# r9y9/deepvoice3_pytorch

Measured on AMD Instinct MI355X. Metric: mel-frames/sec/node (train step, deepvoice3_ljspeech), higher is better.
Workload: dtype f16x3

## Files before the change

deepvoice3_pytorch_amd/csrc/loss.hip:

```cpp
#include "common.h"

namespace {

constexpr int kLossBlock = 256;

__device__ __forceinline__ void block_reduce4(float v[4], float* out ) {
  __shared__ float red[4][4];
#pragma unroll
  for (int k = 0; k < 4; ++k) v[k] = dv3_wave_sum(v[k]);
  const int w = threadIdx.x >> 6;
  if ((threadIdx.x & 63) == 0) {
#pragma unroll
    for (int k = 0; k < 4; ++k) red[w][k] = v[k];
  }
  __syncthreads();
  if (threadIdx.x < 4) out[threadIdx.x] = red[0][threadIdx.x] + red[1][threadIdx.x] +
                                          red[2][threadIdx.x] + red[3][threadIdx.x];
}

template <bool FAST = false>
__device__ __forceinline__ void spec_bd(float yh, float y, float& z, float& dz) {
  const float eps = 1e-8f;
  const float a = yh + eps, b = 1.f - yh + eps;
  constexpr float LN2 = 0.69314718055994530942f;
  const float la = FAST ? __builtin_amdgcn_logf(a) * LN2 : logf(a), lb = FAST ? __builtin_amdgcn_logf(b) * LN2 : logf(b);
  const float ab = a + b;
  z = -y * (la - lb) + ((FAST ? __builtin_amdgcn_logf(ab) * LN2 : logf(ab)) - lb);
  const float ra = __builtin_amdgcn_rcpf(a), rb = __builtin_amdgcn_rcpf(b);
  dz = (a * __builtin_amdgcn_rcpf(ab) - y) * (ra + rb);
}

__device__ __forceinline__ int spec_t_valid(const dv3_spec_loss_desc& p) {
  if (!p.t_valid) return p.T;
  const int tv = p.t_valid[0];
  return tv < p.T ? (tv > p.r ? tv : p.r + 1) : p.T;
}

__device__ __forceinline__ float spec_mask_sum(const dv3_spec_loss_desc& p) {
  float ms = 0.f;
  const int Tr = spec_t_valid(p) - p.r;
  for (int b = 0; b < p.B; ++b) {
    int l = p.lengths[b] - p.r;
    l = l < 0 ? 0 : (l > Tr ? Tr : l);
    ms += (float)l;
  }
  return ms * (float)p.D;
}

__global__ __launch_bounds__(kLossBlock) void spec_loss_kernel(const dv3_spec_loss_desc p) {
  const int Tr = p.T - p.r, D = p.D;
  const int Trv = spec_t_valid(p) - p.r;
  const int64_t n = (int64_t)p.B * Tr * D;
  const bool use_mask = p.w_masked > 0.f && p.lengths;
  const float msum = use_mask ? spec_mask_sum(p) : 1.f;
  const float inv_n = 1.0f / (float)((int64_t)p.B * Trv * D);
  const float wm = use_mask ? p.w_masked : 0.f;
  const float c_all = (1.f - wm) * inv_n, c_msk = use_mask ? wm / msum : 0.f;
  float acc[4] = {0.f, 0.f, 0.f, 0.f};
  const int64_t stride = (int64_t)gridDim.x * kLossBlock;
  const bool t_fast = p.yh_ts < p.yh_ds;
  for (int64_t i = (int64_t)blockIdx.x * kLossBlock + threadIdx.x; i < n; i += stride) {
    int dd, t, b;
    if (t_fast) {
      t = (int)(i % Tr);
      const int64_t bd = i / Tr;
      dd = (int)(bd % D);
      b = (int)(bd / D);
    } else {
      dd = (int)(i % D);
      const int64_t bt = i / D;
      t = (int)(bt % Tr);
      b = (int)(bt / Tr);
    }
    const int64_t ih = b * p.yh_bs + t * p.yh_ts + dd * p.yh_ds;
    const int64_t iy = b * p.y_bs + (int64_t)(t + p.r) * p.y_ts + dd * p.y_ds;
    if (t >= Trv) {
      if (p.dyh) p.dyh[ih] = 0.f;
      continue;
    }
    const float yh = p.y_hat[ih], y = p.y[iy];
    const float m = (use_mask && (t + p.r) < p.lengths[b]) ? 1.f : 0.f;
    const float diff = yh - y;
    const float ad = fabsf(diff);
    acc[0] += ad;
    acc[1] += m * ad;
    float dz = 0.f;
    if (p.w_bd > 0.f) {
      float z;
      spec_bd(yh, y, z, dz);
      acc[2] += z;
      acc[3] += m * z;
    }
    if (p.dyh) {
      const float sgn = (diff > 0.f) ? 1.f : ((diff < 0.f) ? -1.f : 0.f);
      const float coef = c_all + c_msk * m;
      p.dyh[ih] = p.gscale * coef * ((1.f - p.w_bd) * sgn + p.w_bd * dz);
    }
  }
  block_reduce4(acc, p.scratch + (int64_t)blockIdx.x * 4);
}

template <bool FAST>
__global__ __launch_bounds__(kLossBlock) void spec_loss_tiled_kernel(const dv3_spec_loss_desc p, int t_tiles, int d_tiles,
                                                                     int n_tiles) {
  __shared__ float ys[64 * 65];
  const int Tr = p.T - p.r, D = p.D;
  const int Trv = spec_t_valid(p) - p.r;
  const bool use_mask = p.w_masked > 0.f && p.lengths;
  const float msum = use_mask ? spec_mask_sum(p) : 1.f;
  const float inv_n = 1.0f / (float)((int64_t)p.B * Trv * D);
  const float wm = use_mask ? p.w_masked : 0.f;
  const float c_all = (1.f - wm) * inv_n, c_msk = use_mask ? wm / msum : 0.f;
  float acc[4] = {0.f, 0.f, 0.f, 0.f};
  const int tid = threadIdx.x;
  for (int tile = blockIdx.x; tile < n_tiles; tile += gridDim.x) {
    const int dt = tile % d_tiles, tt_ = (tile / d_tiles) % t_tiles, b = tile / (d_tiles * t_tiles);
    const int t0 = tt_ * 64, d0 = dt * 64;
    __syncthreads();
#pragma unroll 4
    for (int q = tid; q < 64 * 64; q += kLossBlock) {
      const int tl = q >> 6, dl = q & 63;
      const int t = t0 + tl, dd = d0 + dl;
      ys[tl * 65 + dl] = (t < Tr && dd < D) ? p.y[b * p.y_bs + (int64_t)(t + p.r) * p.y_ts + dd] : 0.f;
    }
    __syncthreads();
    const int len_b = use_mask ? p.lengths[b] : 0;
#pragma unroll 4
    for (int q = tid; q < 64 * 64; q += kLossBlock) {
      const int dl = q >> 6, tl = q & 63;
      const int t = t0 + tl, dd = d0 + dl;
      if (t >= Tr || dd >= D) continue;
      const int64_t ih = b * p.yh_bs + t + (int64_t)dd * p.yh_ds;
      if (t >= Trv) {
        if (p.dyh) p.dyh[ih] = 0.f;
        continue;
      }
      const float yh = p.y_hat[ih], y = ys[tl * 65 + dl];
      const float m = (use_mask && (t + p.r) < len_b) ? 1.f : 0.f;
      const float diff = yh - y;
      const float ad = fabsf(diff);
      acc[0] += ad;
      acc[1] += m * ad;
      float dz = 0.f;
      if (p.w_bd > 0.f) {
        float z;
        spec_bd<FAST>(yh, y, z, dz);
        acc[2] += z;
        acc[3] += m * z;
      }
      if (p.dyh) {
        const float sgn = (diff > 0.f) ? 1.f : ((diff < 0.f) ? -1.f : 0.f);
        const float coef = c_all + c_msk * m;
        p.dyh[ih] = p.gscale * coef * ((1.f - p.w_bd) * sgn + p.w_bd * dz);
      }
    }
  }
  block_reduce4(acc, p.scratch + (int64_t)blockIdx.x * 4);
}

__global__ __launch_bounds__(256) void spec_loss_tail_zero_kernel(const dv3_spec_loss_desc p) {
  const int64_t n = (int64_t)p.B * p.r * p.D;
  const int64_t i = (int64_t)blockIdx.x * 256 + threadIdx.x;
  if (i >= n) return;
  const int dd = (int)(i % p.D);
  const int64_t bt = i / p.D;
  const int t = p.T - p.r + (int)(bt % p.r);
  const int b = (int)(bt / p.r);
  p.dyh[b * p.yh_bs + t * p.yh_ts + dd * p.yh_ds] = 0.f;
}

__global__ __launch_bounds__(256) void spec_loss_finish_kernel(const dv3_spec_loss_desc p,
                                                               int n_blocks) {
  float acc[4] = {0.f, 0.f, 0.f, 0.f};
  for (int i = threadIdx.x; i < n_blocks; i += 256)
#pragma unroll
    for (int k = 0; k < 4; ++k) acc[k] += p.scratch[(int64_t)i * 4 + k];
  __shared__ float fin[4];
// ... 56 lines not shown
  for (int i = threadIdx.x; i < n_blocks; i += 256) acc[0] += scratch[(int64_t)i * 4];
  __shared__ float fin[4];
  block_reduce4(acc, fin);
  __syncthreads();
  if (threadIdx.x == 0) {
    if (va) {
      int64_t n = count * min(va[0], cap_a);
      if (vb) n *= min(vb[0], cap_b);
      scale = 1.0f / (float)n;
    }
    out1[0] = fin[0] * scale;
  }
}

__device__ __forceinline__ float bce_elem(float x, float y) {
  const float lx = fmaxf(logf(x), -100.f), l1x = fmaxf(logf(1.f - x), -100.f);
  return -(y * lx + (1.f - y) * l1x);
}

__global__ __launch_bounds__(256) void bce_kernel(const float* __restrict__ p,
                                                  const float* __restrict__ t,
                                                  float* __restrict__ dp, float* __restrict__ scratch,
                                                  int64_t n, float gscale, int T = 0,
                                                  const int32_t* __restrict__ t_valid = nullptr) {
  float acc[4] = {0.f, 0.f, 0.f, 0.f};
  const int Tv = t_valid ? min(t_valid[0], T) : T;
  const float inv_n = 1.0f / (float)(t_valid ? (n / T) * Tv : n);
  const int64_t stride = (int64_t)gridDim.x * 256;
  for (int64_t i = (int64_t)blockIdx.x * 256 + threadIdx.x; i < n; i += stride) {
    if (t_valid && (int)(i % T) >= Tv) {
      if (dp) dp[i] = 0.f;
      continue;
    }
    const float x = p[i], y = t[i];
    acc[0] += bce_elem(x, y);
    if (dp) dp[i] = gscale * inv_n * (x - y) / fmaxf((1.f - x) * x, 1e-12f);
  }
  block_reduce4(acc, scratch + (int64_t)blockIdx.x * 4);
}


constexpr int kItemSliceFrames = 64, kItemMaxSlices = 64;

inline int item_slices(int T) {
  const int s = dv3_cdiv(T, kItemSliceFrames);
  return s < 1 ? 1 : (s > kItemMaxSlices ? kItemMaxSlices : s);
}

__device__ __forceinline__ int clamp_len(int l, int cap) { return l < 0 ? 0 : (l > cap ? cap : l); }

__device__ __forceinline__ void item_slice(int n, int& t0, int& t1) {
  const int per = (n + (int)gridDim.x - 1) / (int)gridDim.x;
  t0 = min((int)blockIdx.x * per, n);
  t1 = min(t0 + per, n);
}

template <bool FAST>
__global__ __launch_bounds__(kLossBlock) void spec_items_kernel(const dv3_spec_items_desc p) {
  const int b = blockIdx.y, D = p.D;
  int t0, t1;
  item_slice(clamp_len(p.lengths[b] - p.r, p.T - p.r), t0, t1);
// ... 75 lines not shown
template <class Desc>
inline bool spec_time_fast(const Desc& d) {
  return d.yh_ts == 1 && d.y_ds == 1 && d.yh_ds > 1 && d.y_ts > 1 && (int64_t)d.B * d.yh_bs < (1ll << 40);
}

inline int loss_blocks(int64_t n) {
  int64_t b = dv3_cdiv64(n, (int64_t)kLossBlock * 4);
  if (b < 1) b = 1;
  if (b > 1024) b = 1024;
  return (int)b;
}

}

int g_loss_fast_log = 1;

extern "C" int dv3_spec_loss_scratch_floats(int32_t B, int32_t T, int32_t D) {
  int64_t tiles = (int64_t)B * dv3_cdiv(T, 64) * dv3_cdiv(D, 64);
  if (tiles > 1024) tiles = 1024;
  const int64_t flat = loss_blocks((int64_t)B * T * D);
  return (int)(4 * (tiles > flat ? tiles : flat) + 16);
}

extern "C" int dv3_spec_loss_f32(const dv3_spec_loss_desc* d, void* stream) {
  DV3_REQUIRE(d && d->y_hat && d->y && d->out4 && d->scratch, "spec_loss: null pointer");
  DV3_REQUIRE(d->B > 0 && d->D > 0 && d->r >= 0 && d->T > d->r, "spec_loss: bad dims");
  DV3_REQUIRE(d->w_masked <= 0.f || d->lengths, "spec_loss: masked weight needs lengths");
  hipStream_t st = (hipStream_t)stream;
  const int64_t n = (int64_t)d->B * (d->T - d->r) * d->D;
  int nb = loss_blocks(n);
  if (spec_time_fast(*d)) {
    const int t_tiles = dv3_cdiv(d->T - d->r, 64), d_tiles = dv3_cdiv(d->D, 64);
    const int64_t nt = (int64_t)d->B * t_tiles * d_tiles;
    nb = (int)(nt < 1024 ? nt : 1024);
    if (g_loss_fast_log) hipLaunchKernelGGL(spec_loss_tiled_kernel<true>, dim3(nb), dim3(kLossBlock), 0, st, *d, t_tiles, d_tiles, (int)nt);
    else hipLaunchKernelGGL(spec_loss_tiled_kernel<false>, dim3(nb), dim3(kLossBlock), 0, st, *d, t_tiles, d_tiles, (int)nt);
  } else {
    hipLaunchKernelGGL(spec_loss_kernel, dim3(nb), dim3(kLossBlock), 0, st, *d);
  }
  if (d->dyh && d->r > 0) {
    const int64_t nt = (int64_t)d->B * d->r * d->D;
    hipLaunchKernelGGL(spec_loss_tail_zero_kernel, dim3((unsigned)dv3_cdiv64(nt, 256)), dim3(256), 0,
                       st, *d);
  }
  hipLaunchKernelGGL(spec_loss_finish_kernel, dim3(1), dim3(256), 0, st, *d, nb);
  return dv3_check_launch("spec_loss_f32");
}

extern "C" int dv3_guided_attn_loss_f32(const float* attn, const int32_t* in_len,
                                        const int32_t* out_len, float* dattn, float* out1,
                                        float* scratch, int32_t L, int32_t B, int32_t Tq, int32_t Tk,
                                        float g, float gscale, void* stream) {
  DV3_REQUIRE(attn && in_len && out_len && out1 && scratch, "guided_attn: null pointer");
  DV3_REQUIRE(L > 0 && B > 0 && Tq > 0 && Tk > 0 && g > 0.f, "guided_attn: bad dims");
  hipStream_t st = (hipStream_t)stream;
  const int64_t per = (int64_t)B * Tq * Tk;
  const int nb = loss_blocks(per);
  hipLaunchKernelGGL(guided_attn_kernel, dim3(nb), dim3(256), 0, st, attn, in_len, out_len, dattn,
                     scratch, L, B, Tq, Tk, g, gscale, (const int32_t*)nullptr, (const int32_t*)nullptr);
  hipLaunchKernelGGL(sum_finish_kernel, dim3(1), dim3(256), 0, st, scratch, nb,
                     1.0f / (float)(per * L), out1, (const int32_t*)nullptr, 0, (const int32_t*)nullptr, 0, (int64_t)0);
  return dv3_check_launch("guided_attn_loss_f32");
}

extern "C" int dv3_guided_attn_loss_valid_f32(const float* attn, const int32_t* in_len, const int32_t* out_len,
                                              float* dattn, float* out1, float* scratch, int32_t L, int32_t B,
                                              int32_t Tq, int32_t Tk, float g, float gscale,
                                              const int32_t* tq_valid, const int32_t* tk_valid, void* stream) {
  DV3_REQUIRE(attn && in_len && out_len && out1 && scratch && tq_valid && tk_valid, "guided_attn_valid: null pointer");
// ... 9 lines not shown
}

extern "C" int dv3_bce_loss_f32(const float* p, const float* t, float* dp, float* out1,
                                float* scratch, int64_t n, float gscale, void* stream) {
  DV3_REQUIRE(p && t && out1 && scratch && n > 0, "bce_loss: bad args");
  hipStream_t st = (hipStream_t)stream;
  const int nb = loss_blocks(n);
  hipLaunchKernelGGL(bce_kernel, dim3(nb), dim3(256), 0, st, p, t, dp, scratch, n, gscale, 0, (const int32_t*)nullptr);
  hipLaunchKernelGGL(sum_finish_kernel, dim3(1), dim3(256), 0, st, scratch, nb, 1.0f / (float)n, out1,
                     (const int32_t*)nullptr, 0, (const int32_t*)nullptr, 0, (int64_t)0);
  return dv3_check_launch("bce_loss_f32");
}

extern "C" int dv3_bce_loss_valid_f32(const float* p, const float* t, float* dp, float* out1, float* scratch,
                                      int64_t rows, int32_t T, const int32_t* t_valid, float gscale, void* stream) {
  DV3_REQUIRE(p && t && out1 && scratch && t_valid && rows > 0 && T > 0, "bce_loss_valid: bad args");
  hipStream_t st = (hipStream_t)stream;
  const int64_t n = rows * T;
  const int nb = loss_blocks(n);
  hipLaunchKernelGGL(bce_kernel, dim3(nb), dim3(256), 0, st, p, t, dp, scratch, n, gscale, (int)T, t_valid);
  hipLaunchKernelGGL(sum_finish_kernel, dim3(1), dim3(256), 0, st, scratch, nb, 0.f, out1, t_valid, (int)T,
                     (const int32_t*)nullptr, 0, rows);
  return dv3_check_launch("bce_loss_valid_f32");
}

extern "C" int dv3_loss_items_scratch_floats(int32_t B, int32_t T) {
  if (B <= 0 || T <= 0) return 0;
  return (int)((int64_t)4 * B * item_slices(T));
}

extern "C" int dv3_spec_loss_items_f32(const dv3_spec_items_desc* d, void* stream) {
  DV3_REQUIRE(d && d->y_hat && d->y && d->lengths && d->out && d->scratch, "spec_loss_items: null pointer");
  DV3_REQUIRE(d->B > 0 && d->B <= 65535 && d->D > 0 && d->r >= 0 && d->T > 0, "spec_loss_items: bad dims");
  hipStream_t st = (hipStream_t)stream;
  const int Tr = d->T > d->r ? d->T - d->r : 0;
  const int S = Tr > 0 ? item_slices(Tr) : 0;
  if (S > 0) {
    DV3_REQUIRE((int64_t)dv3_cdiv(Tr, S) * d->D < (1ll << 31), "spec_loss_items: slice too large");
    if (spec_time_fast(*d) && g_loss_fast_log)
      hipLaunchKernelGGL(spec_items_kernel<true>, dim3(S, d->B), dim3(kLossBlock), 0, st, *d);
    else
      hipLaunchKernelGGL(spec_items_kernel<false>, dim3(S, d->B), dim3(kLossBlock), 0, st, *d);
  }
  hipLaunchKernelGGL(items_finish_kernel, dim3(dv3_cdiv(d->B, 256)), dim3(256), 0, st, (const float*)d->scratch, (int)d->B,
                     S, 2, d->out, d->lengths, (int)d->r, Tr, (const int32_t*)nullptr, 0, (int64_t)d->D);
  return dv3_check_launch("spec_loss_items_f32");
// ... 29 lines not shown
```

deepvoice3_pytorch_amd/ops.py:

```python
import contextlib
import ctypes
import functools
import math

import torch

from . import _lib
from ._lib import CONSTS, STRUCTS, _env_flag, _env_int, _env_str

EPI_LINEAR = CONSTS["DV3_EPI_LINEAR"]
EPI_RELU = CONSTS["DV3_EPI_RELU"]
EPI_SIGMOID = CONSTS["DV3_EPI_SIGMOID"]
EPI_GLU = CONSTS["DV3_EPI_GLU"]
EPI_HIGHWAY = CONSTS["DV3_EPI_HIGHWAY"]
EPI_DGRAD = CONSTS["DV3_EPI_DGRAD"]
EPI_SOFTSIGN = CONSTS["DV3_EPI_SOFTSIGN"]
STORE_BCT = CONSTS["DV3_STORE_BCT"]
STORE_INTERLEAVE2 = CONSTS["DV3_STORE_INTERLEAVE2"]

_conv_desc = STRUCTS["dv3_conv_desc"]
_wgrad_desc = STRUCTS["dv3_wgrad_desc"]
_wn_desc = STRUCTS["dv3_wn_desc"]
_wn_bwd_desc = STRUCTS["dv3_wn_bwd_desc"]
_gate_bwd_desc = STRUCTS["dv3_gate_bwd_desc"]
# ... 1030 lines not shown


fuse_gate_bwd = _env_flag("DV3_FUSE_GATE", True)
fuse_gate_max_elems = _env_int("DV3_FUSE_GATE_MAX", 4 << 20)
pair_words = _env_flag("DV3_PAIR_WORDS", True)
gate_fuse_stats = {"fused": 0, "standalone": 0}


class _GateToken(object):
    __slots__ = ("ab", "mode", "residual", "x", "C", "pair")

    def __init__(self, ab, mode, residual, x, C, pair):
        self.ab, self.mode, self.residual, self.x, self.C, self.pair = ab, mode, residual, x, C, pair


class _GateResult(object):
    __slots__ = ("tok", "dab", "dres", "part", "n_part", "pair", "version")

    def __init__(self, tok, gate, version):
        self.tok, self.dab, self.dres, self.part, self.n_part = tok, gate.dab, gate.dres, gate.part, gate.n_part
        self.pair, self.version = gate.pair, version


def mark_sole_consumer(y):
    if fuse_gate_bwd and getattr(y, "_dv3_tok", None) is not None:
        y._dv3_sole = True
    return y


def _spk_strides(spk):
    if spk is None:
        return 0, 0, 0
    if spk.dim() == 2:
        return spk.stride(0), 1, 0
    return spk.stride(0), spk.stride(1), 1


def _grads_in_place(leaves):
    return all(getattr(t, "_dv3_grad_inplace", False) and t.grad is not None and t.requires_grad for t in leaves)


def _grad_inplace_arm(ctx, v, g, bias):
    leaves = [t for t in (v, g, bias) if t is not None]
    ctx.inplace = bool(leaves) and _grads_in_place(leaves)
    ctx.leaves = (v, g, bias) if ctx.inplace else None
    if ctx.inplace:
# ... 86 lines not shown
            raise ValueError("gated layers keep the sequence length")
        ab_dtype = torch.bfloat16 if (_gemm_mode == "bf16" and pk.fwd_s is not None and split_only) else torch.float32
        ab = torch.empty((B, M, T), dtype=ab_dtype, device=x.device) if (gated and need_grad) else None
        if spk is not None:
            spk = _c(spk)
        res_in = x if gated else (_c(r) if r is not None else None)
        r2c = _c(r2) if r2 is not None else None
        y = conv_gemm(x, pk.fwd, pk.lda, pk.a_half, B=B, Cin=Cin, Tin=T, M=M, Tout=Tout,
                      J=J_, dil=cfg.dil, padL=padL, mode=mode, Cg=Cg,
                      bias=bias, spk=spk, spk_strides=_spk_strides(spk),
                      r=res_in if (mode == EPI_HIGHWAY or cfg.residual or not gated) else None,
                      r2=r2c, residual=int(cfg.residual), ab=ab, xmask=bits, xmask_rs=bits_rs, xmask_c8=keep8,
                      drop_scale=dscale, a_split=pk.fwd_s if _gemm_mode != "f32" else None,
                      store_mode=STORE_INTERLEAVE2 if cfg.transposed else STORE_BCT)
        if need_grad:
            _grad_inplace_arm(ctx, v, g, bias)
            ctx.cfg, ctx.pk, ctx.dims = cfg, pk, (B, Cin, T, Tout, M, Cg, J, padL)
            ctx.bits, ctx.bits_rs, ctx.dscale = bits, bits_rs, dscale
            ctx.spk_dim = spk.dim() if spk is not None else 0
            ctx.has_r, ctx.has_r2 = (r is not None), (r2 is not None)
            ctx.has_bias = bias is not None
            ctx.save_for_backward(x, v, g, ab if gated else y)
            ctx.tok = ctx.prod = None
            split_modes = _gemm_mode in ("f16x3", "bf16x3")
            ctx.pair_ok = bool(gated and pair_words and split_modes and pk.bwd_s is not None and
                               split_only and ab.dtype == torch.float32 and (spk is None or spk.dim() == 2) and
                               not (M <= 64 and Cin <= 64))
            if fuse_gate_bwd and split_modes and pk.bwd_s is not None:
                if gated and ab.dtype == torch.float32 and spk is None and split_only and \
                        B * Cg * T <= fuse_gate_max_elems:
                    ctx.tok = _GateToken(ab, mode, int(cfg.residual), x if mode == EPI_HIGHWAY else None, Cg,
                                         pair=ctx.pair_ok)
                    y._dv3_tok = ctx.tok
                prod = getattr(x_in, "_dv3_tok", None) if (x_in is x and getattr(x_in, "_dv3_sole", False)) else None
                if prod is not None and prod.C == Cin and ctx.needs_input_grad[0] and Tout == T and \
                        (J_ - 1) * cfg.dil <= 64 and J_ <= 16:
                    ctx.prod = prod
        return y

    @staticmethod
    def backward(ctx, dy):
        cfg, pk = ctx.cfg, ctx.pk
        B, Cin, T, Tout, M, Cg, J, padL = ctx.dims
        x, v, g, saved = ctx.saved_tensors
        mode = cfg.mode
        gated = mode in (EPI_GLU, EPI_HIGHWAY)
        dy = _c(dy)
        rs2 = math.sqrt(0.5)
        dr = dr2 = dspk = None
        r_scale = 0.0
        n_part, g_pair, part_t = B, False, False
        if gated:
            glu_skip = mode == EPI_GLU and cfg.residual
            fused = getattr(dy, "_dv3_gate", None)
            if fused is not None and ctx.tok is not None and fused.tok is ctx.tok and dy._version == fused.version:
                dab, dres, part = fused.dab, fused.dres, fused.part
                n_part, g_pair, part_t = fused.n_part, fused.pair, True
                dy._dv3_gate = None
                gate_fuse_stats["fused"] += 1
            else:
                g_pair = ctx.pair_ok
                dab, dres, part = gate_bwd(dy, saved, x if mode == EPI_HIGHWAY else None, B=B, C=Cg, T=T,
                                           mode=mode, residual=int(cfg.residual), want_dres=(mode == EPI_HIGHWAY),
                                           pair=g_pair)
                gate_fuse_stats["standalone"] += 1
            if glu_skip:
                dres, r_scale = dy, rs2
            if ctx.spk_dim == 2:
                dspk = part[:, :Cg].contiguous()
            elif ctx.spk_dim == 3:
                dspk = dab[:, :Cg, :]
            gmat, Tg = dab, T
        elif cfg.transposed:
            O = pk.O
            _, _, part = gate_bwd(dy, None, None, B=B, C=O, T=2 * T, mode=EPI_LINEAR, want_dpre=False)
# ... 724 lines not shown
        d.y_bs, d.y_ts, d.y_ds = y.stride()
        d.dyh, d.out4, d.scratch = _ptr(dyh), out4.data_ptr(), scratch.data_ptr()
        d.B, d.T, d.D, d.r = B, T, D, r
        d.w_masked, d.w_bd, d.gscale = w_masked, w_bd, 1.0
        d.t_valid = _ptr(t_valid)
        _lib.call("dv3_spec_loss_f32", ctypes.byref(d), _stream())
        ctx.dyh = dyh
        return out4

    @staticmethod
    def backward(ctx, dout):
        g = ctx.dyh * dout[2] if ctx.dyh is not None else None
        return g, None, None, None, None, None, None


def spec_loss(y_hat, y, lengths, r=1, w_masked=0.5, w_bd=0.1, t_valid=None):
    return SpecLossFn.apply(y_hat, y, lengths, r, w_masked, w_bd, t_valid)


class _NoCtx(object):
    needs_input_grad = (True,)


def spec_loss_with_grad(y_hat, y, lengths, r=1, w_masked=0.5, w_bd=0.1, t_valid=None):
    c = _NoCtx()
    out4 = SpecLossFn.forward(c, y_hat.detach(), y, lengths, r, w_masked, w_bd, t_valid)
    return out4, c.dyh


def guided_attention_loss_with_grad(attn, in_len, out_len, g=0.2, tq_valid=None, tk_valid=None):
    c = _NoCtx()
    out1 = GuidedAttnLossFn.forward(c, attn.detach(), in_len, out_len, g, tq_valid, tk_valid)
    return out1, c.dattn


def bce_loss_with_grad(p, t, t_valid=None):
    c = _NoCtx()
    out1 = BCELossFn.forward(c, p.detach(), t, t_valid)
    return out1, c.dp


def sum_scalars(a, b, c=None, d=None):
    out = torch.empty(1, dtype=torch.float32, device=a.device)
    _lib.call("dv3_sum_scalars_f32", a.data_ptr(), b.data_ptr(), _ptr(c), _ptr(d), out.data_ptr(), _stream())
    return out


def scaled_copy(a, alpha=1.0):
    out = torch.empty_like(a)
    _lib.call("dv3_axpby_f32", a.data_ptr(), None, out.data_ptr(), a.numel(), float(alpha), _stream())
    return out


class GuidedAttnLossFn(torch.autograd.Function):
    @staticmethod
    def forward(ctx, attn, in_len, out_len, g, tq_valid=None, tk_valid=None):
        attn = _c(_chk(attn, "attn"))
        L, B, Tq, Tk = attn.shape
        dev = attn.device
        out1 = torch.empty(1, dtype=torch.float32, device=dev)
        scratch = torch.empty(4 * 1024 + 16, dtype=torch.float32, device=dev)
        dattn = torch.empty_like(attn) if ctx.needs_input_grad[0] else None
# ... 135 lines not shown
```

deepvoice3_pytorch_amd/torch_ops.py:

```python
import math

import torch

from . import ops

_NS = "dv3hip"
_lib = torch.library.Library(_NS, "DEF")

GLU, HIGHWAY = 0, 1
ACT_LINEAR, ACT_RELU, ACT_SIGMOID = 0, 1, 2
_MODES = {GLU: ops.EPI_GLU, HIGHWAY: ops.EPI_HIGHWAY}
_ACTS = {ACT_LINEAR: ops.EPI_LINEAR, ACT_RELU: ops.EPI_RELU, ACT_SIGMOID: ops.EPI_SIGMOID}


class _Ctx(object):

    def __init__(self, needs):
        self.needs_input_grad = tuple(needs)
        self.saved_tensors = ()

    def save_for_backward(self, *tensors):
        self.saved_tensors = tensors


# ... 274 lines not shown

def _attn_backward(ctx, g_ctx, g_P, g_Pd, g_bits):
    q, k, v, P, Pd, bits = ctx.saved_tensors
    if g_ctx is None:
        g_ctx = torch.zeros_like(q)
    dq, dk, dv = torch.ops.dv3hip.attention_bwd(g_ctx.contiguous(), g_P, q, k, v, P, Pd, bits, ctx.p_drop)
    return dq, dk, dv, None, None, None, None


torch.library.register_autograd("dv3hip::attention_fwd", _attn_backward, setup_context=_attn_setup)


_lib.define("sincos_pos_embed(Tensor positions, Tensor table, float w) -> Tensor")
_lib.impl("sincos_pos_embed", lambda positions, table, w: ops.sincos_pos_bct(positions, table, float(w)), "CUDA")
_lib.impl("sincos_pos_embed", lambda positions, table, w: table.new_empty((positions.shape[0], table.shape[1],
                                                                           positions.shape[1])), "Meta")


_lib.define("spec_loss_fwd(Tensor y_hat, Tensor y, Tensor? lengths, int r, float w_masked, float w_bd) "
            "-> (Tensor out4, Tensor grad_y_hat)")
_lib.define("guided_attn_loss_fwd(Tensor attn, Tensor in_lens, Tensor out_lens, float g) -> (Tensor loss, Tensor grad_attn)")
_lib.define("bce_loss_fwd(Tensor p, Tensor target) -> (Tensor loss, Tensor grad_p)")
_lib.impl("spec_loss_fwd", lambda y_hat, y, lengths, r, w_masked, w_bd: ops.spec_loss_with_grad(y_hat, y, lengths, r, w_masked,
                                                                                                 w_bd), "CUDA")
_lib.impl("guided_attn_loss_fwd", lambda attn, il, ol, g: ops.guided_attention_loss_with_grad(attn, il, ol, g), "CUDA")
_lib.impl("bce_loss_fwd", lambda p, t: ops.bce_loss_with_grad(p, t), "CUDA")
_lib.impl("spec_loss_fwd", lambda y_hat, y, lengths, r, w_masked, w_bd: (y_hat.new_empty((4,)), torch.empty_like(y_hat)), "Meta")
_lib.impl("guided_attn_loss_fwd", lambda attn, il, ol, g: (attn.new_empty((1,)), torch.empty_like(attn)), "Meta")
_lib.impl("bce_loss_fwd", lambda p, t: (p.new_empty((1,)), torch.empty_like(p)), "Meta")


def _loss_setup(ctx, inputs, output):
    ctx.save_for_backward(output[1])


def _spec_backward(ctx, g_out4, g_grad):
    (gr,) = ctx.saved_tensors
    return gr * g_out4[2], None, None, None, None, None


def _scalar_backward(n_inputs):
    def backward(ctx, g_loss, g_grad):
        (gr,) = ctx.saved_tensors
        return (gr * g_loss,) + (None,) * (n_inputs - 1)
    return backward


torch.library.register_autograd("dv3hip::spec_loss_fwd", _spec_backward, setup_context=_loss_setup)
torch.library.register_autograd("dv3hip::guided_attn_loss_fwd", _scalar_backward(4), setup_context=_loss_setup)
# ... 44 lines not shown
```

include/dv3hip.h:

```cpp
#ifndef DV3HIP_H
#define DV3HIP_H

#include <stdint.h>

#ifdef __cplusplus
extern "C" {
#endif

#define DV3_OK 0
#define DV3_EINVAL (-1)
#define DV3_ELAUNCH (-2)

#define DV3_ABI_VERSION 49
int dv3_abi_version(void);
const char* dv3_last_error(void);
int dv3_device_info(int dev, char* name, int name_len, int* n_cu);
int dv3_sizeof(const char* name);
int dv3_debug_set(int what, int value);
int dv3_debug_read(int what, void* dst, int64_t bytes);
int dv3_debug_get(int what);

int dv3_ring_standin(const void* src, int64_t src_bytes, void* scratch, int64_t scratch_bytes, int64_t bytes,
                     int32_t channels, int32_t threads, float bytes_per_us, void* stream);

// ... 233 lines not shown
                                 int32_t n_pos, int32_t apply_sincos, void* stream);
int dv3_sincos_pos_bwd_f32(const int64_t* pos, const float* table, const float* w,
                           int32_t w_per_batch, const float* dout, float* dw, int32_t B, int32_t T,
                           int32_t C, int32_t n_pos, void* stream);
int dv3_sincos_pos_bwd2_f32(const int64_t* pos, const float* table, const float* w,
                            int32_t w_per_batch, const float* dout, float* partial, int32_t n_chunks, float* dw,
                            int32_t B, int32_t T, int32_t C, int32_t n_pos, void* stream);
int dv3_shift_append_f32(float* buf, const float* x, int64_t rows, int32_t L, int64_t x_stride,
                         void* stream);
int dv3_ragged_pad_rows_b32(const uint32_t* src, const int32_t* row_off, uint32_t* out, int32_t B,
                            int32_t T_out, int32_t D, int32_t lead, int32_t t_stride, void* stream);
int dv3_deinterleave2_f32(const float* dy, float* out, int32_t B, int32_t O, int32_t T,
                          void* stream);

typedef struct dv3_spec_loss_desc {
  const float* y_hat; const float* y; const int32_t* lengths;
  float* dyh; float* out4; float* scratch;
  int64_t yh_bs, yh_ts, yh_ds;
  int64_t y_bs, y_ts, y_ds;
  int32_t B, T, D, r; float w_masked, w_bd, gscale;
  const int32_t* t_valid;
} dv3_spec_loss_desc;
int dv3_spec_loss_f32(const dv3_spec_loss_desc* d, void* stream);
int dv3_spec_loss_scratch_floats(int32_t B, int32_t T, int32_t D);

int dv3_guided_attn_loss_f32(const float* attn, const int32_t* in_len, const int32_t* out_len,
                             float* dattn, float* out1, float* scratch, int32_t L, int32_t B,
                             int32_t Tq, int32_t Tk, float g, float gscale, void* stream);
int dv3_guided_attn_loss_valid_f32(const float* attn, const int32_t* in_len, const int32_t* out_len,
                                   float* dattn, float* out1, float* scratch, int32_t L, int32_t B,
                                   int32_t Tq, int32_t Tk, float g, float gscale, const int32_t* tq_valid,
                                   const int32_t* tk_valid, void* stream);
int dv3_bce_loss_f32(const float* p, const float* t, float* dp, float* out1, float* scratch,
                     int64_t n, float gscale, void* stream);
int dv3_bce_loss_valid_f32(const float* p, const float* t, float* dp, float* out1, float* scratch,
                           int64_t rows, int32_t T, const int32_t* t_valid, float gscale, void* stream);

typedef struct dv3_spec_items_desc {
  const float* y_hat; const float* y; const int32_t* lengths;
  float* out; float* scratch;
  int64_t yh_bs, yh_ts, yh_ds;
  int64_t y_bs, y_ts, y_ds;
  int32_t B, T, D, r;
} dv3_spec_items_desc;
int dv3_loss_items_scratch_floats(int32_t B, int32_t T);
int dv3_spec_loss_items_f32(const dv3_spec_items_desc* d, void* stream);
int dv3_bce_loss_items_f32(const float* p, const float* t, const int32_t* lengths, float* out, float* scratch,
                           int32_t B, int32_t T, void* stream);
int dv3_guided_attn_loss_items_f32(const float* attn, const int32_t* in_len, const int32_t* out_len, float* out,
                                   float* scratch, int32_t L, int32_t B, int32_t Tq, int32_t Tk, float g,
                                   void* stream);

int dv3_grad_sqnorm_f32(const float* g, int64_t n, float* partial, int32_t n_partial,
                        float* out2, void* stream);
int dv3_clip_adam_f32(float* p, const float* g, float* m, float* v, int64_t n,
                      const float* grad_norm, float clip, const float* hyper, float beta1,
                      float beta2, float eps, float weight_decay, float grad_prescale,
                      void* stream);

// ... 150 lines not shown
```

Baseline: 3.808 million.

## Fuse sigmoid-head backward into spec and BCE loss kernels

Adds head variants of the spectrogram and BCE loss kernels. These compute the gradient with respect to the pre-sigmoid activation directly (dL/dy * y(1-y)) and optionally write per-tile bias partial sums. The sigmoid-epilogue GEMM backward picks up this precomputed gradient through a token, so the standalone dy materialisation and the sigmoid-gate backward pass are skipped. The tiled spec-loss kernel is also restructured to prefetch the next tile into registers while the current one computes. This adds token bookkeeping and a fallback redo path when the upstream gradient is not the placeholder, with extra complexity and risk of silent mismatches.

```diff
diff --git a/deepvoice3_pytorch_amd/csrc/loss.hip b/deepvoice3_pytorch_amd/csrc/loss.hip
--- a/deepvoice3_pytorch_amd/csrc/loss.hip
+++ b/deepvoice3_pytorch_amd/csrc/loss.hip
@@ -4,7 +4,11 @@
 
 constexpr int kLossBlock = 256;
 
-__device__ __forceinline__ void block_reduce4(float v[4], float* out ) {
+struct spec_loss_args : dv3_spec_loss_desc {
+  float* dpre; float* bias_part;
+};
+
+__device__ __forceinline__ void block_reduce4(float v[4], float* out , float* extra = nullptr) {
   __shared__ float red[4][4];
 #pragma unroll
   for (int k = 0; k < 4; ++k) v[k] = dv3_wave_sum(v[k]);
@@ -14,8 +18,16 @@
     for (int k = 0; k < 4; ++k) red[w][k] = v[k];
   }
   __syncthreads();
-  if (threadIdx.x < 4) out[threadIdx.x] = red[0][threadIdx.x] + red[1][threadIdx.x] +
-                                          red[2][threadIdx.x] + red[3][threadIdx.x];
+  if (threadIdx.x < 4) {
+    const float sum = red[0][threadIdx.x] + red[1][threadIdx.x] + red[2][threadIdx.x] + red[3][threadIdx.x];
+    out[threadIdx.x] = sum;
+    if (extra && threadIdx.x == 1) extra[0] = sum;
+  }
+}
+
+__device__ __forceinline__ float sigmoid_head_dz(float dyh, float yh) {
+  const float d = dyh * 1.0f;
+  return d * yh * (1.0f - yh);
 }
 
 template <bool FAST = false>
@@ -47,7 +59,7 @@
   return ms * (float)p.D;
 }
 
-__global__ __launch_bounds__(kLossBlock) void spec_loss_kernel(const dv3_spec_loss_desc p) {
+__global__ __launch_bounds__(kLossBlock) void spec_loss_kernel(const spec_loss_args p) {
   const int Tr = p.T - p.r, D = p.D;
   const int Trv = spec_t_valid(p) - p.r;
   const int64_t n = (int64_t)p.B * Tr * D;
@@ -76,6 +88,7 @@
     const int64_t iy = b * p.y_bs + (int64_t)(t + p.r) * p.y_ts + dd * p.y_ds;
     if (t >= Trv) {
       if (p.dyh) p.dyh[ih] = 0.f;
+      if (p.dpre) p.dpre[ih] = 0.f;
       continue;
     }
     const float yh = p.y_hat[ih], y = p.y[iy];
@@ -91,17 +104,42 @@
       acc[2] += z;
       acc[3] += m * z;
     }
-    if (p.dyh) {
+    if (p.dyh || p.dpre) {
       const float sgn = (diff > 0.f) ? 1.f : ((diff < 0.f) ? -1.f : 0.f);
       const float coef = c_all + c_msk * m;
-      p.dyh[ih] = p.gscale * coef * ((1.f - p.w_bd) * sgn + p.w_bd * dz);
+      const float g = p.gscale * coef * ((1.f - p.w_bd) * sgn + p.w_bd * dz);
+      if (p.dyh) p.dyh[ih] = g;
+      if (p.dpre) p.dpre[ih] = sigmoid_head_dz(g, yh);
+    }
+  }
+  if (p.dpre) {
+    const int64_t nz = (int64_t)p.B * p.r * D;
+    for (int64_t i = (int64_t)blockIdx.x * kLossBlock + threadIdx.x; i < nz; i += stride) {
+      const int dd = (int)(i % D);
+      const int64_t bt = i / D;
+      const int64_t ih = (bt / p.r) * p.yh_bs + (Tr + (bt % p.r)) * p.yh_ts + dd * p.yh_ds;
+      p.dpre[ih] = 0.f;
+      if (p.dyh) p.dyh[ih] = 0.f;
     }
   }
   block_reduce4(acc, p.scratch + (int64_t)blockIdx.x * 4);
 }
 
-template <bool FAST>
-__global__ __launch_bounds__(kLossBlock) void spec_loss_tiled_kernel(const dv3_spec_loss_desc p, int t_tiles, int d_tiles,
+__global__ __launch_bounds__(256) void spec_head_rowsum_kernel(const spec_loss_args p, int t_tiles) {
+  const int64_t n = (int64_t)p.B * t_tiles * p.D;
+  const int64_t i = (int64_t)blockIdx.x * 256 + threadIdx.x;
+  if (i >= n) return;
+  const int dd = (int)(i % p.D);
+  const int64_t bt = i / p.D;
+  const int tt = (int)(bt % t_tiles), b = (int)(bt / t_tiles);
+  const int t1 = min(tt * 64 + 64, p.T - p.r);
+  float s[8] = {0.f, 0.f, 0.f, 0.f, 0.f, 0.f, 0.f, 0.f};
+  for (int t = tt * 64; t < t1; ++t) s[t & 7] += p.dpre[b * p.yh_bs + t * p.yh_ts + dd * p.yh_ds];
+  p.bias_part[(int64_t)dd * ((int64_t)p.B * t_tiles) + bt] = ((s[0] + s[1]) + (s[2] + s[3])) + ((s[4] + s[5]) + (s[6] + s[7]));
+}
+
+template <bool FAST, bool HEAD>
+__global__ __launch_bounds__(kLossBlock) void spec_loss_tiled_kernel(const spec_loss_args p, int t_tiles, int d_tiles,
                                                                      int n_tiles) {
   __shared__ float ys[64 * 65];
   const int Tr = p.T - p.r, D = p.D;
@@ -113,46 +151,104 @@
   const float c_all = (1.f - wm) * inv_n, c_msk = use_mask ? wm / msum : 0.f;
   float acc[4] = {0.f, 0.f, 0.f, 0.f};
   const int tid = threadIdx.x;
+  const int tl = tid & 63, dw = tid >> 6;
+  const bool sums = HEAD && p.bias_part != nullptr;
+  const int64_t n_part = (int64_t)p.B * t_tiles;
+  float tg[16], yv[16];
+  auto fetch = [&](int tile) {
+    const int dt = tile % d_tiles, tt_ = (tile / d_tiles) % t_tiles, b = tile / (d_tiles * t_tiles);
+    const int t0 = tt_ * 64, d0 = dt * 64;
+    const int dd = d0 + tl;
+    const float* __restrict__ yp = p.y + b * p.y_bs + (int64_t)(t0 + dw + p.r) * p.y_ts + dd;
+#pragma unroll
+    for (int k = 0; k < 16; ++k) tg[k] = (t0 + dw + 4 * k < Tr && dd < D) ? yp[(int64_t)(4 * k) * p.y_ts] : 0.f;
+    const int t = t0 + tl;
+    const float* __restrict__ hp = p.y_hat + b * p.yh_bs + t + (int64_t)(d0 + dw) * p.yh_ds;
+#pragma unroll
+    for (int k = 0; k < 16; ++k) yv[k] = (t < Trv && d0 + dw + 4 * k < D) ? hp[(int64_t)(4 * k) * p.yh_ds] : 0.f;
+  };
+  if ((int)blockIdx.x < n_tiles) fetch(blockIdx.x);
   for (int tile = blockIdx.x; tile < n_tiles; tile += gridDim.x) {
     const int dt = tile % d_tiles, tt_ = (tile / d_tiles) % t_tiles, b = tile / (d_tiles * t_tiles);
     const int t0 = tt_ * 64, d0 = dt * 64;
+    const int nd = min(64, D - d0);
     __syncthreads();
-#pragma unroll 4
-    for (int q = tid; q < 64 * 64; q += kLossBlock) {
-      const int tl = q >> 6, dl = q & 63;
-      const int t = t0 + tl, dd = d0 + dl;
-      ys[tl * 65 + dl] = (t < Tr && dd < D) ? p.y[b * p.y_bs + (int64_t)(t + p.r) * p.y_ts + dd] : 0.f;
-    }
+#pragma unroll
+    for (int k = 0; k < 16; ++k) ys[(dw + 4 * k) * 65 + tl] = tg[k];
+    float yc[16];
+#pragma unroll
+    for (int k = 0; k < 16; ++k) yc[k] = yv[k];
+    if (tile + (int)gridDim.x < n_tiles) fetch(tile + gridDim.x);
     __syncthreads();
     const int len_b = use_mask ? p.lengths[b] : 0;
-#pragma unroll 4
-    for (int q = tid; q < 64 * 64; q += kLossBlock) {
-      const int dl = q >> 6, tl = q & 63;
-      const int t = t0 + tl, dd = d0 + dl;
-      if (t >= Tr || dd >= D) continue;
-      const int64_t ih = b * p.yh_bs + t + (int64_t)dd * p.yh_ds;
-      if (t >= Trv) {
-        if (p.dyh) p.dyh[ih] = 0.f;
-        continue;
+    const int t = t0 + tl;
+    const float m = (use_mask && (t + p.r) < len_b) ? 1.f : 0.f;
+    const float coef = c_all + c_msk * m;
+    const int64_t ih0 = b * p.yh_bs + t + (int64_t)(d0 + dw) * p.yh_ds;
+    const int64_t ihs = 4 * p.yh_ds;
+    if (t < Trv) {
+#pragma unroll
+      for (int k = 0; k < 16; ++k) {
+        const int dl = dw + 4 * k;
+        if (dl >= nd) break;
+        const int64_t ih = ih0 + k * ihs;
+        const float yh = yc[k], y = ys[tl * 65 + dl];
+        const float diff = yh - y;
+        const float ad = fabsf(diff);
+        acc[0] += ad;
+        acc[1] += m * ad;
+        float dz = 0.f;
+        if (p.w_bd > 0.f) {
+          float z;
+          spec_bd<FAST>(yh, y, z, dz);
+          acc[2] += z;
+          acc[3] += m * z;
+        }
+        if (p.dyh || HEAD) {
+          const float sgn = (diff > 0.f) ? 1.f : ((diff < 0.f) ? -1.f : 0.f);
+          const float g = p.gscale * coef * ((1.f - p.w_bd) * sgn + p.w_bd * dz);
+          if (p.dyh) p.dyh[ih] = g;
+          if (HEAD) {
+            const float gz = sigmoid_head_dz(g, yh);
+            p.dpre[ih] = gz;
+            if (sums) ys[tl * 65 + dl] = gz;
+          }
+        }
       }
-      const float yh = p.y_hat[ih], y = ys[tl * 65 + dl];
-      const float m = (use_mask && (t + p.r) < len_b) ? 1.f : 0.f;
-      const float diff = yh - y;
-      const float ad = fabsf(diff);
-      acc[0] += ad;
-      acc[1] += m * ad;
-      float dz = 0.f;
-      if (p.w_bd > 0.f) {
-        float z;
-        spec_bd<FAST>(yh, y, z, dz);
-        acc[2] += z;
-        acc[3] += m * z;
+    } else {
+      if (t < Tr) {
+        int64_t ih = ih0;
+        for (int dl = dw; dl < nd; dl += 4, ih += ihs) {
+          if (p.dyh) p.dyh[ih] = 0.f;
+          if (HEAD) p.dpre[ih] = 0.f;
+        }
       }
-      if (p.dyh) {
-        const float sgn = (diff > 0.f) ? 1.f : ((diff < 0.f) ? -1.f : 0.f);
-        const float coef = c_all + c_msk * m;
-        p.dyh[ih] = p.gscale * coef * ((1.f - p.w_bd) * sgn + p.w_bd * dz);
+      if (sums)
+        for (int dl = dw; dl < nd; dl += 4) ys[tl * 65 + dl] = 0.f;
+    }
+    if (HEAD && tt_ == t_tiles - 1) {
+      for (int tz = Tr + tl; tz < p.T; tz += 64) {
+        int64_t ih = b * p.yh_bs + tz + (int64_t)(d0 + dw) * p.yh_ds;
+        for (int dl = dw; dl < nd; dl += 4, ih += ihs) {
+          p.dpre[ih] = 0.f;
+          if (p.dyh) p.dyh[ih] = 0.f;
+        }
       }
+    }
+    if (sums) {
+      __syncthreads();
+      const int bin = tid >> 2, part = tid & 3;
+      float v[16];
+#pragma unroll
+      for (int i = 0; i < 16; ++i) v[i] = ys[(part * 16 + i) * 65 + bin];
+#pragma unroll
+      for (int w = 1; w < 16; w <<= 1)
+#pragma unroll
+        for (int i = 0; i < 16; i += 2 * w) v[i] += v[i + w];
+      float s = v[0];
+      s += __shfl_xor(s, 1, 4);
+      s += __shfl_xor(s, 2, 4);
+      if (part == 0 && bin < nd) p.bias_part[(int64_t)(d0 + bin) * n_part + (int64_t)b * t_tiles + tt_] = s;
     }
   }
   block_reduce4(acc, p.scratch + (int64_t)blockIdx.x * 4);
@@ -255,7 +351,9 @@
                                                   const float* __restrict__ t,
                                                   float* __restrict__ dp, float* __restrict__ scratch,
                                                   int64_t n, float gscale, int T = 0,
-                                                  const int32_t* __restrict__ t_valid = nullptr) {
+                                                  const int32_t* __restrict__ t_valid = nullptr,
+                                                  float* __restrict__ dpre = nullptr,
+                                                  float* __restrict__ bias_part = nullptr) {
   float acc[4] = {0.f, 0.f, 0.f, 0.f};
   const int Tv = t_valid ? min(t_valid[0], T) : T;
   const float inv_n = 1.0f / (float)(t_valid ? (n / T) * Tv : n);
@@ -263,13 +361,22 @@
   for (int64_t i = (int64_t)blockIdx.x * 256 + threadIdx.x; i < n; i += stride) {
     if (t_valid && (int)(i % T) >= Tv) {
       if (dp) dp[i] = 0.f;
+      if (dpre) dpre[i] = 0.f;
       continue;
     }
     const float x = p[i], y = t[i];
     acc[0] += bce_elem(x, y);
-    if (dp) dp[i] = gscale * inv_n * (x - y) / fmaxf((1.f - x) * x, 1e-12f);
-  }
-  block_reduce4(acc, scratch + (int64_t)blockIdx.x * 4);
+    if (dp || dpre) {
+      const float g = gscale * inv_n * (x - y) / fmaxf((1.f - x) * x, 1e-12f);
+      if (dp) dp[i] = g;
+      if (dpre) {
+        const float gz = sigmoid_head_dz(g, x);
+        dpre[i] = gz;
+        acc[1] += gz;
+      }
+    }
+  }
+  block_reduce4(acc, scratch + (int64_t)blockIdx.x * 4, bias_part ? bias_part + blockIdx.x : nullptr);
 }
 
 
@@ -391,29 +498,48 @@
   return (int)(4 * (tiles > flat ? tiles : flat) + 16);
 }
 
-extern "C" int dv3_spec_loss_f32(const dv3_spec_loss_desc* d, void* stream) {
+static int spec_loss_launch(const dv3_spec_loss_desc* d, float* dpre, float* bias_part, void* stream) {
   DV3_REQUIRE(d && d->y_hat && d->y && d->out4 && d->scratch, "spec_loss: null pointer");
   DV3_REQUIRE(d->B > 0 && d->D > 0 && d->r >= 0 && d->T > d->r, "spec_loss: bad dims");
   DV3_REQUIRE(d->w_masked <= 0.f || d->lengths, "spec_loss: masked weight needs lengths");
   hipStream_t st = (hipStream_t)stream;
+  spec_loss_args a;
+  static_cast<dv3_spec_loss_desc&>(a) = *d;
+  a.dpre = dpre;
+  a.bias_part = bias_part;
   const int64_t n = (int64_t)d->B * (d->T - d->r) * d->D;
   int nb = loss_blocks(n);
   if (spec_time_fast(*d)) {
     const int t_tiles = dv3_cdiv(d->T - d->r, 64), d_tiles = dv3_cdiv(d->D, 64);
     const int64_t nt = (int64_t)d->B * t_tiles * d_tiles;
     nb = (int)(nt < 1024 ? nt : 1024);
-    if (g_loss_fast_log) hipLaunchKernelGGL(spec_loss_tiled_kernel<true>, dim3(nb), dim3(kLossBlock), 0, st, *d, t_tiles, d_tiles, (int)nt);
-    else hipLaunchKernelGGL(spec_loss_tiled_kernel<false>, dim3(nb), dim3(kLossBlock), 0, st, *d, t_tiles, d_tiles, (int)nt);
+    auto k = dpre ? (g_loss_fast_log ? spec_loss_tiled_kernel<true, true> : spec_loss_tiled_kernel<false, true>)
+                     : (g_loss_fast_log ? spec_loss_tiled_kernel<true, false> : spec_loss_tiled_kernel<false, false>);
+    hipLaunchKernelGGL(k, dim3(nb), dim3(kLossBlock), 0, st, a, t_tiles, d_tiles, (int)nt);
   } else {
-    hipLaunchKernelGGL(spec_loss_kernel, dim3(nb), dim3(kLossBlock), 0, st, *d);
-  }
-  if (d->dyh && d->r > 0) {
+    hipLaunchKernelGGL(spec_loss_kernel, dim3(nb), dim3(kLossBlock), 0, st, a);
+    if (dpre && bias_part) {
+      const int t_tiles = dv3_cdiv(d->T - d->r, 64);
+      const int64_t ns = (int64_t)d->B * t_tiles * d->D;
+      hipLaunchKernelGGL(spec_head_rowsum_kernel, dim3((unsigned)dv3_cdiv64(ns, 256)), dim3(256), 0, st, a, t_tiles);
+    }
+  }
+  if (d->dyh && !dpre && d->r > 0) {
     const int64_t nt = (int64_t)d->B * d->r * d->D;
     hipLaunchKernelGGL(spec_loss_tail_zero_kernel, dim3((unsigned)dv3_cdiv64(nt, 256)), dim3(256), 0,
                        st, *d);
   }
   hipLaunchKernelGGL(spec_loss_finish_kernel, dim3(1), dim3(256), 0, st, *d, nb);
   return dv3_check_launch("spec_loss_f32");
+}
+
+extern "C" int dv3_spec_loss_f32(const dv3_spec_loss_desc* d, void* stream) {
+  return spec_loss_launch(d, nullptr, nullptr, stream);
+}
+
+extern "C" int dv3_spec_loss_head_f32(const dv3_spec_loss_desc* d, float* dpre, float* bias_part, void* stream) {
+  DV3_REQUIRE(dpre, "spec_loss_head: dpre is required");
+  return spec_loss_launch(d, dpre, bias_part, stream);
 }
 
 extern "C" int dv3_guided_attn_loss_f32(const float* attn, const int32_t* in_len,
@@ -469,6 +595,28 @@
   hipLaunchKernelGGL(sum_finish_kernel, dim3(1), dim3(256), 0, st, scratch, nb, 0.f, out1, t_valid, (int)T,
                      (const int32_t*)nullptr, 0, rows);
   return dv3_check_launch("bce_loss_valid_f32");
+}
+
+extern "C" int dv3_bce_loss_head_parts(int64_t n) { return n > 0 ? loss_blocks(n) : 0; }
+
+extern "C" int dv3_bce_loss_head_f32(const float* p, const float* t, float* dp, float* dpre, float* bias_part, float* out1,
+                                     float* scratch, int64_t rows, int32_t T, const int32_t* t_valid, float gscale,
+                                     void* stream) {
+  DV3_REQUIRE(p && t && dpre && out1 && scratch && rows > 0 && T > 0, "bce_loss_head: bad args");
+  hipStream_t st = (hipStream_t)stream;
+  const int64_t n = rows * T;
+  const int nb = loss_blocks(n);
+  if (t_valid) {
+    hipLaunchKernelGGL(bce_kernel, dim3(nb), dim3(256), 0, st, p, t, dp, scratch, n, gscale, (int)T, t_valid, dpre, bias_part);
+    hipLaunchKernelGGL(sum_finish_kernel, dim3(1), dim3(256), 0, st, scratch, nb, 0.f, out1, t_valid, (int)T,
+                       (const int32_t*)nullptr, 0, rows);
+  } else {
+    hipLaunchKernelGGL(bce_kernel, dim3(nb), dim3(256), 0, st, p, t, dp, scratch, n, gscale, 0, (const int32_t*)nullptr, dpre,
+                       bias_part);
+    hipLaunchKernelGGL(sum_finish_kernel, dim3(1), dim3(256), 0, st, scratch, nb, 1.0f / (float)n, out1,
+                       (const int32_t*)nullptr, 0, (const int32_t*)nullptr, 0, (int64_t)0);
+  }
+  return dv3_check_launch("bce_loss_head_f32");
 }
 
 extern "C" int dv3_loss_items_scratch_floats(int32_t B, int32_t T) {
diff --git a/deepvoice3_pytorch_amd/ops.py b/deepvoice3_pytorch_amd/ops.py
--- a/deepvoice3_pytorch_amd/ops.py
+++ b/deepvoice3_pytorch_amd/ops.py
@@ -1076,6 +1076,55 @@
         self.pair, self.version = gate.pair, version
 
 
+fuse_loss_head = _env_flag("DV3_FUSE_LOSS_HEAD", True)
+loss_head_stats = {"fused": 0, "standalone": 0}
+_head_dummy = {}
+
+
+class _HeadToken(object):
+    __slots__ = ("shape", "result")
+
+    def __init__(self, shape):
+        self.shape, self.result = tuple(shape), None
+
+
+class _HeadResult(object):
+    __slots__ = ("dz", "version", "redo")
+
+    def __init__(self, dz, redo):
+        self.dz, self.version, self.redo = dz, dz._version, redo
+
+
+def _head_stand_in(shape, device):
+    z = _head_dummy.get(device)
+    if z is None:
+        z = _head_dummy[device] = torch.zeros(1, dtype=torch.float32, device=device)
+    return z.expand(*shape)
+
+
+def _is_head_stand_in(dy):
+    z = _head_dummy.get(dy.device)
+    return z is not None and dy.data_ptr() == z.data_ptr() and z._version == 0 and \
+        all(st == 0 or n == 1 for n, st in zip(dy.shape, dy.stride()))
+
+
+def _loss_head_token(y_hat, transposed_only):
+    if not fuse_loss_head or y_hat.dtype != torch.float32:
+        return None, None
+    tok = getattr(y_hat, "_dv3_head", None)
+    if tok is not None and not transposed_only and tuple(y_hat.shape) == tok.shape and y_hat.is_contiguous():
+        return tok, "self"
+    base = getattr(y_hat, "_base", None)
+    tok = getattr(base, "_dv3_head", None) if base is not None else None
+    if tok is None or y_hat.dim() != 3 or tuple(base.shape) != tok.shape or not base.is_contiguous():
+        return None, None
+    B, M, T = tok.shape
+    if tuple(y_hat.shape) == (B, T, M) and y_hat.data_ptr() == base.data_ptr() and \
+            all(n == 1 or st == want for n, st, want in zip(y_hat.shape, y_hat.stride(), (M * T, 1, T))):
+        return tok, "t"
+    return None, None
+
+
 def mark_sole_consumer(y):
     if fuse_gate_bwd and getattr(y, "_dv3_tok", None) is not None:
         y._dv3_sole = True
@@ -1208,6 +1257,9 @@
             ctx.has_bias = bias is not None
             ctx.save_for_backward(x, v, g, ab if gated else y)
             ctx.tok = ctx.prod = None
+            ctx.head = None
+            if fuse_loss_head and mode == EPI_SIGMOID and r is None and r2 is None and not cfg.transposed:
+                ctx.head = y._dv3_head = _HeadToken(y.shape)
             split_modes = _gemm_mode in ("f16x3", "bf16x3")
             ctx.pair_ok = bool(gated and pair_words and split_modes and pk.bwd_s is not None and
                                split_only and ab.dtype == torch.float32 and (spk is None or spk.dim() == 2) and
@@ -1231,12 +1283,27 @@
         x, v, g, saved = ctx.saved_tensors
         mode = cfg.mode
         gated = mode in (EPI_GLU, EPI_HIGHWAY)
-        dy = _c(dy)
+        head, tok = None, getattr(ctx, "head", None)
+        if tok is not None:
+            head, tok.result = tok.result, None
+            if head is not None:
+                if tuple(dy.shape) == tuple(head.dz.shape) and _is_head_stand_in(dy) and head.dz._version == head.version:
+                    dy = None
+                else:
+                    dy = head.redo().view(head.dz.shape) + dy
+                    head = None
+            loss_head_stats["fused" if head is not None else "standalone"] += 1
+        if dy is not None:
+            dy = _c(dy)
         rs2 = math.sqrt(0.5)
         dr = dr2 = dspk = None
         r_scale = 0.0
         n_part, g_pair, part_t = B, False, False
-        if gated:
+        if head is not None:
+            gmat = head.dz
+            _, _, part = gate_bwd(gmat, None, None, B=B, C=M, T=Tout, mode=EPI_LINEAR, want_dpre=False)
+            dres, Tg = None, Tout
+        elif gated:
             glu_skip = mode == EPI_GLU and cfg.residual
             fused = getattr(dy, "_dv3_gate", None)
             if fused is not None and ctx.tok is not None and fused.tok is ctx.tok and dy._version == fused.version:
@@ -2007,10 +2074,36 @@
     needs_input_grad = (True,)
 
 
-def spec_loss_with_grad(y_hat, y, lengths, r=1, w_masked=0.5, w_bd=0.1, t_valid=None):
-    c = _NoCtx()
-    out4 = SpecLossFn.forward(c, y_hat.detach(), y, lengths, r, w_masked, w_bd, t_valid)
-    return out4, c.dyh
+def spec_loss_with_grad(y_hat, y, lengths, r=1, w_masked=0.5, w_bd=0.1, t_valid=None, head=None):
+    tok, how = _loss_head_token(y_hat, True) if head is not False else (None, None)
+    yd = y_hat.detach()
+    if tok is None:
+        c = _NoCtx()
+        out4 = SpecLossFn.forward(c, yd, y, lengths, r, w_masked, w_bd, t_valid)
+        return out4, c.dyh
+    y = _dense_or_copy(_chk(y, "y"))
+    B, T, D = yd.shape
+    dev = yd.device
+    out4 = torch.empty(4, dtype=torch.float32, device=dev)
+    scratch = torch.empty(_lib.lib().dv3_spec_loss_scratch_floats(B, T, D), dtype=torch.float32, device=dev)
+    dz = torch.empty((B, D, T), dtype=torch.float32, device=dev)
+    d = _spec_loss_desc()
+    d.y_hat, d.y, d.lengths = yd.data_ptr(), y.data_ptr(), _ptr(lengths)
+    d.yh_bs, d.yh_ts, d.yh_ds = D * T, 1, T
+    d.y_bs, d.y_ts, d.y_ds = y.stride()
+    d.dyh, d.out4, d.scratch = None, out4.data_ptr(), scratch.data_ptr()
+    d.B, d.T, d.D, d.r = B, T, D, r
+    d.w_masked, d.w_bd, d.gscale = w_masked, w_bd, 1.0
+    d.t_valid = _ptr(t_valid)
+    _lib.call("dv3_spec_loss_head_f32", ctypes.byref(d), dz.data_ptr(), None, _stream())
+
+    def redo():
+        c = _NoCtx()
+        SpecLossFn.forward(c, yd, y, lengths, r, w_masked, w_bd, t_valid)
+        return c.dyh.transpose(1, 2)
+
+    tok.result = _HeadResult(dz, redo)
+    return out4, _head_stand_in(yd.shape, dev)
 
 
 def guided_attention_loss_with_grad(attn, in_len, out_len, g=0.2, tq_valid=None, tk_valid=None):
@@ -2019,10 +2112,29 @@
     return out1, c.dattn
 
 
-def bce_loss_with_grad(p, t, t_valid=None):
-    c = _NoCtx()
-    out1 = BCELossFn.forward(c, p.detach(), t, t_valid)
-    return out1, c.dp
+def bce_loss_with_grad(p, t, t_valid=None, head=None):
+    tok, how = _loss_head_token(p, False) if head is not False else (None, None)
+    pd = p.detach()
+    if tok is None or tok.shape[1] != 1 or not pd.is_contiguous() or (t_valid is not None and how != "t"):
+        c = _NoCtx()
+        out1 = BCELossFn.forward(c, pd, t, t_valid)
+        return out1, c.dp
+    t = _c(_chk(t, "t"))
+    B, _, T = tok.shape
+    dev = pd.device
+    out1 = torch.empty(1, dtype=torch.float32, device=dev)
+    scratch = torch.empty(4 * 1024 + 16, dtype=torch.float32, device=dev)
+    dz = torch.empty(tok.shape, dtype=torch.float32, device=dev)
+    _lib.call("dv3_bce_loss_head_f32", pd.data_ptr(), t.data_ptr(), None, dz.data_ptr(), None, out1.data_ptr(),
+              scratch.data_ptr(), B, T, _ptr(t_valid), 1.0, _stream())
+
+    def redo():
+        c = _NoCtx()
+        BCELossFn.forward(c, pd, t, t_valid)
+        return c.dp
+
+    tok.result = _HeadResult(dz, redo)
+    return out1, _head_stand_in(pd.shape, dev)
 
 
 def sum_scalars(a, b, c=None, d=None):
diff --git a/deepvoice3_pytorch_amd/torch_ops.py b/deepvoice3_pytorch_amd/torch_ops.py
--- a/deepvoice3_pytorch_amd/torch_ops.py
+++ b/deepvoice3_pytorch_amd/torch_ops.py
@@ -320,9 +320,9 @@
 _lib.define("guided_attn_loss_fwd(Tensor attn, Tensor in_lens, Tensor out_lens, float g) -> (Tensor loss, Tensor grad_attn)")
 _lib.define("bce_loss_fwd(Tensor p, Tensor target) -> (Tensor loss, Tensor grad_p)")
 _lib.impl("spec_loss_fwd", lambda y_hat, y, lengths, r, w_masked, w_bd: ops.spec_loss_with_grad(y_hat, y, lengths, r, w_masked,
-                                                                                                 w_bd), "CUDA")
+                                                                                                 w_bd, head=False), "CUDA")
 _lib.impl("guided_attn_loss_fwd", lambda attn, il, ol, g: ops.guided_attention_loss_with_grad(attn, il, ol, g), "CUDA")
-_lib.impl("bce_loss_fwd", lambda p, t: ops.bce_loss_with_grad(p, t), "CUDA")
+_lib.impl("bce_loss_fwd", lambda p, t: ops.bce_loss_with_grad(p, t, head=False), "CUDA")
 _lib.impl("spec_loss_fwd", lambda y_hat, y, lengths, r, w_masked, w_bd: (y_hat.new_empty((4,)), torch.empty_like(y_hat)), "Meta")
 _lib.impl("guided_attn_loss_fwd", lambda attn, il, ol, g: (attn.new_empty((1,)), torch.empty_like(attn)), "Meta")
 _lib.impl("bce_loss_fwd", lambda p, t: (p.new_empty((1,)), torch.empty_like(p)), "Meta")
diff --git a/include/dv3hip.h b/include/dv3hip.h
--- a/include/dv3hip.h
+++ b/include/dv3hip.h
@@ -279,6 +279,7 @@
   const int32_t* t_valid;
 } dv3_spec_loss_desc;
 int dv3_spec_loss_f32(const dv3_spec_loss_desc* d, void* stream);
+int dv3_spec_loss_head_f32(const dv3_spec_loss_desc* d, float* dpre, float* bias_part, void* stream);
 int dv3_spec_loss_scratch_floats(int32_t B, int32_t T, int32_t D);
 
 int dv3_guided_attn_loss_f32(const float* attn, const int32_t* in_len, const int32_t* out_len,
@@ -292,6 +293,11 @@
                      int64_t n, float gscale, void* stream);
 int dv3_bce_loss_valid_f32(const float* p, const float* t, float* dp, float* out1, float* scratch,
                            int64_t rows, int32_t T, const int32_t* t_valid, float gscale, void* stream);
+
+int dv3_bce_loss_head_f32(const float* p, const float* t, float* dp, float* dpre, float* bias_part, float* out1,
+                          float* scratch, int64_t rows, int32_t T, const int32_t* t_valid, float gscale,
+                          void* stream);
+int dv3_bce_loss_head_parts(int64_t n);
 
 typedef struct dv3_spec_items_desc {
   const float* y_hat; const float* y; const int32_t* lengths;
```

Measured after the change: 3.856 million (median of 6 runs). +1.3%, better.
